# nikhil-lalgudi/distributed-llm-alignment

Measured on AMD Instinct MI355X. Metric: preference-samples/sec (whole node), Llama-3-8B DPO at 1/2/4/8 MI355X, higher is better.
Workload: dtype bf16; 1 GPU; model=llama3-8b, global_batch=16, seq_len=1024, parallelism=dp1, micro_batch_pairs=4, grad_accum=4, ref_model=frozen, co-resident, backend=single-process, gemm_selection=tunableop:off

## Files before the change

### distributed_llm_alignment_amd/csrc/attention.hip

```cpp
#include <cstdlib>
#include <stdexcept>
#include <type_traits>
#include "common.h"

#include <cstring>
#include "attn_params.h"

namespace dla {

typedef __attribute__((address_space(3))) s16x4 lds_s16x4;

template <int D>
constexpr int attn_dp() { return (D + 31) / 32 * 32; }

template <int W>
__device__ __forceinline__ int swz(int row, int ch) {
  constexpr int NCH = W / 8;
  constexpr int MASK = (NCH & (NCH - 1)) == 0 ? NCH - 1 : 3;
  const int f = (((row & 3) << 2) | ((row >> 2) & 3)) & MASK;
  return row * W + ((ch ^ f) << 3);
}

__device__ __forceinline__ int ds_swz(int row) { return (row >> 1) & 7; }
__device__ __forceinline__ int ds_off(int row, int c4) { return row * 32 + ((c4 ^ ds_swz(row)) << 2); }
// ... 1232 lines not shown
      bf16_t* dkp = p.dk + b * p.dk_sb + kj * p.dk_st + static_cast<int64_t>(hk) * p.dk_sh;
      bf16_t* dvp = p.dv + b * p.dv_sb + kj * p.dv_st + static_cast<int64_t>(hk) * p.dv_sh;
      auto store_row = [&](bf16_t* dst, f32x16 x, float sc, int dt) {
#pragma unroll
        for (int g4 = 0; g4 < 4; g4 += 2) {
          const uint32_t a0 = pack2bf(x[4 * g4] * sc, x[4 * g4 + 1] * sc);
          const uint32_t a1 = pack2bf(x[4 * g4 + 2] * sc, x[4 * g4 + 3] * sc);
          const uint32_t c0 = pack2bf(x[4 * g4 + 4] * sc, x[4 * g4 + 5] * sc);
          const uint32_t c1 = pack2bf(x[4 * g4 + 6] * sc, x[4 * g4 + 7] * sc);
          const auto r0 = __builtin_amdgcn_permlane32_swap(a0, c0, false, false);
          const auto r1 = __builtin_amdgcn_permlane32_swap(a1, c1, false, false);
          if (32 * dt + 8 * g4 + 8 * h < D)
            *reinterpret_cast<uint4*>(dst + 32 * dt + 8 * g4 + 8 * h) = make_uint4(r0[0], r1[0], r0[1], r1[1]);
        }
      };
      if (D == 80 && p.rope_cos != nullptr) {
        const int pos = p.rope_pos ? p.rope_pos[static_cast<int64_t>(b) * p.Tk + kj] : kj;
        store_row(dkp, unrotate_tile0_rot32(dk[j][0], p.rope_cos + static_cast<int64_t>(pos) * 16 + 4 * h,
                                            p.rope_sin + static_cast<int64_t>(pos) * 16 + 4 * h),
                  p.scale, 0);
#pragma unroll
        for (int dt = 1; dt < DT; ++dt) store_row(dkp, dk[j][dt], p.scale, dt);
      } else if (DP == D && p.rope_cos != nullptr) {
        const int pos = p.rope_pos ? p.rope_pos[static_cast<int64_t>(b) * p.Tk + kj] : kj;
        const float* cp = p.rope_cos + static_cast<int64_t>(pos) * (D / 2) + 4 * h;
        const float* sp = p.rope_sin + static_cast<int64_t>(pos) * (D / 2) + 4 * h;
#pragma unroll
        for (int dt = 0; dt < DT / 2; ++dt) {
          f32x16 lo = dk[j][dt], hi = dk[j][dt + DT / 2];
#pragma unroll
          for (int g = 0; g < 4; ++g) {
            const f32x4 c4 = *reinterpret_cast<const f32x4*>(cp + 32 * dt + 8 * g);
            const f32x4 s4 = *reinterpret_cast<const f32x4*>(sp + 32 * dt + 8 * g);
#pragma unroll
            for (int e = 0; e < 4; ++e) {
              const float a = lo[4 * g + e], bb = hi[4 * g + e];
              lo[4 * g + e] = a * c4[e] + bb * s4[e];
              hi[4 * g + e] = bb * c4[e] - a * s4[e];
            }
          }
          store_row(dkp, lo, p.scale, dt);
          store_row(dkp, hi, p.scale, dt + DT / 2);
        }
      } else {
#pragma unroll
        for (int dt = 0; dt < DT; ++dt) store_row(dkp, dk[j][dt], p.scale, dt);
      }
#pragma unroll
      for (int dt = 0; dt < DT; ++dt) store_row(dvp, dv[j][dt], 1.f, dt);
    } else {
      const int64_t off = ((static_cast<int64_t>(sidx) * p.B + b) * p.Tk + kj) * p.Hkv * D +
                          static_cast<int64_t>(hk) * D;
      float* dkp = p.dk_part + off;
      float* dvp = p.dv_part + off;
#pragma unroll
      for (int dt = 0; dt < DT; ++dt) {
#pragma unroll
        for (int g4 = 0; g4 < 4; ++g4) {
          const int d = 32 * dt + 8 * g4 + 4 * h;
          if (d >= D) continue;
          *reinterpret_cast<f32x4*>(dkp + d) = f32x4{dk[j][dt][4 * g4], dk[j][dt][4 * g4 + 1],
                                                     dk[j][dt][4 * g4 + 2], dk[j][dt][4 * g4 + 3]};
          *reinterpret_cast<f32x4*>(dvp + d) = f32x4{dv[j][dt][4 * g4], dv[j][dt][4 * g4 + 1],
                                                     dv[j][dt][4 * g4 + 2], dv[j][dt][4 * g4 + 3]};
        }
      }
    }
  }
}

#ifdef DLA_BWD_TRACE
__device__ long long g_bwd_trace[8 * 64 * 8];
#define BWD_TS(k)                                                                         \
  do {                                                                                    \
    if (blockIdx.x == DLA_BWD_TRACE && lane == 0 && it < 64)                              \
      g_bwd_trace[(w * 64 + it) * 8 + (k)] = static_cast<long long>(__builtin_amdgcn_s_memtime()); \
  } while (0)
#else
#define BWD_TS(k) \
  do {            \
  } while (0)
#endif

template <int D, bool CAUSAL>
__global__ __launch_bounds__(512) void attn_bwd8_kernel(AttnBwdParams p) {
  constexpr int BKV = kAttnBwdKeys, BQ = kAttnBwdQRows, NT = 512;
  constexpr int DP = attn_dp<D>();
  constexpr int NCH = DP / 8;
  constexpr int NCHL = D / 8;
  constexpr int KS = D / 16;
  constexpr int DT = DP / 32;
  constexpr int NDS = D / 16;
  constexpr bool Q_EXACT = BQ * NCH == NT;
  static_assert(BQ * NCH <= NT && (BKV * NCH) % NT == 0 && BKV == 256 && BQ == 32, "tile geometry");
  __shared__ __attribute__((aligned(16))) bf16_t lds[2 * BQ * DP + BKV * BQ + 2 * BKV * DP];
  bf16_t* const Qs = lds;
  bf16_t* const dOs = lds + BQ * DP;
  bf16_t* const dSs = lds + 2 * BQ * DP;
  bf16_t* const Ks = dSs + BKV * BQ;
  bf16_t* const Vs = Ks + BKV * DP;

  const int tid = threadIdx.x, lane = tid & 63, w = __builtin_amdgcn_readfirstlane(tid >> 6);
  const int l32 = lane & 31, h = lane >> 5;
  const int group = p.Hq / p.Hkv;
  const int hpb = group / p.hsplit;
  const int nrest = p.Hkv * p.B * p.hsplit;
  const int kb = static_cast<int>(blockIdx.x) / nrest;
  int rest = static_cast<int>(blockIdx.x) - kb * nrest;
  const int sidx = rest % p.hsplit;
  rest /= p.hsplit;
  const int hk = rest % p.Hkv, b = rest / p.Hkv;
  const int k0 = kb * BKV;
  const int kw = k0 + 32 * w;
  const int kbeg = p.kv_start ? p.kv_start[b] : 0;
  const int kend = p.kv_end ? p.kv_end[b] : p.Tk;

  const bool rope_in = p.rope_inputs != 0;
  {
    const bf16_t* kp = p.k + b * p.k_sb + static_cast<int64_t>(hk) * p.k_sh;
    const bf16_t* vp = p.v + b * p.v_sb + static_cast<int64_t>(hk) * p.v_sh;
#pragma unroll 2
    for (int c = 0; c < BKV * NCH / NT; ++c) {
      const int ci = tid + NT * c;
      const int row = ci / NCH, ch = ci % NCH;
      const int key = k0 + row;
      const bool in = key < p.Tk && ch < NCHL;
      bf16x8 kv = in ? load_bf16x8(kp + key * p.k_st + ch * 8) : bf16x8{};
      if constexpr (DP == D) {
        if (rope_in)
          kv = rope_rot_chunk<NCH>(kv, ch, in, static_cast<int64_t>(b) * p.Tk + key, key, p.rope_cos,
                                   p.rope_sin, p.rope_pos);
      }
      store_bf16x8(Ks + swz<DP>(row, ch), kv);
      store_bf16x8(Vs + swz<DP>(row, ch), in ? load_bf16x8(vp + key * p.v_st + ch * 8) : bf16x8{});
    }
  }

  int qt0, qend;
  bwd_q_range<CAUSAL>(k0, p.Tq, p.causal_off, p.window, qt0, qend);
  const int nqt = (qend - qt0 + BQ - 1) / BQ;
  const bool block_has_keys = k0 < kend && k0 + BKV > kbeg;
  const int n_iter = block_has_keys ? hpb * nqt : 0;
  const int hq0 = hk * group + sidx * hpb;

  const int qrow = tid / NCH, qch = tid % NCH;
  const bool qslot = (Q_EXACT || tid < BQ * NCH) && qch < NCHL;
  const uint32_t qlo = static_cast<uint32_t>(qrow * p.q_st + qch * 8) * 2u;
  const uint32_t dlo = static_cast<uint32_t>(qrow * p.do_st + qch * 8) * 2u;
  bf16x8 qreg, dreg;
  auto gld = [](const bf16_t* base, uint32_t off) {
    return load_bf16x8(reinterpret_cast<const bf16_t*>(reinterpret_cast<const char*>(base) + off));
  };
  const int qtend = qt0 + nqt * BQ;
  auto advance = [&](int& hq, int& qt) {
    qt += BQ;
    if (qt >= qtend) {
      qt = qt0;
      ++hq;
    }
  };
  auto prefetch = [&](int hq, int qt) {
    const bf16_t* qp = p.q + b * p.q_sb + static_cast<int64_t>(hq) * p.q_sh;
    const bf16_t* dop = p.dout + b * p.do_sb + static_cast<int64_t>(hq) * p.do_sh;
    if (!qslot) {
      qreg = bf16x8{};
      dreg = bf16x8{};
    } else if (qt + BQ <= p.Tq) {
      qreg = gld(qp + static_cast<int64_t>(qt) * p.q_st, qlo);
      dreg = gld(dop + static_cast<int64_t>(qt) * p.do_st, dlo);
    } else {
      const int qq = min(qt + qrow, p.Tq - 1);
      const bf16x8 a = load_bf16x8(qp + qq * p.q_st + qch * 8);
      const bf16x8 g = load_bf16x8(dop + qq * p.do_st + qch * 8);
      const bool in = qt + qrow < p.Tq;
      qreg = in ? a : bf16x8{};
      dreg = in ? g : bf16x8{};
    }
  };
  auto stage = [&]() {
    if (Q_EXACT || tid < BQ * NCH) {
      store_bf16x8(Qs + swz<DP>(qrow, qch), qreg);
      store_bf16x8(dOs + swz<DP>(qrow, qch), dreg);
    }
  };

  const int i16 = lane & 15, qq = i16 >> 2, pp = i16 & 3, half16 = (lane >> 4) & 1, g4l = lane >> 4;
  constexpr int FMASK = (NCH & (NCH - 1)) == 0 ? NCH - 1 : 3;
  auto swzf = [](int row) { return (((row & 3) << 2) | ((row >> 2) & 3)) & FMASK; };
  int rq = l32 * DP, rx = h ^ swzf(l32);
  const int c1 = 2 * half16 + (pp >> 1);
  int tq0 = (4 * h + qq) * DP + (pp & 1) * 4, tx0 = c1 ^ swzf(4 * h + qq);
  int tq1 = (4 * h + 8 + qq) * DP + (pp & 1) * 4, tx1 = c1 ^ swzf(4 * h + 8 + qq);
  int wq = l32 * 32, wx = h ^ ds_swz(l32);
  constexpr int DQT = NDS == 4 ? 1 : 2;
  const int dslice = NDS == 4 ? (w & 3) : w;
  const int dthalf = NDS == 4 ? (w >> 2) : 0;
  int qoff[DQT][2], koff[2];
#pragma unroll
  for (int t = 0; t < DQT; ++t) {
    const int tt = NDS == 4 ? dthalf : t;
    qoff[t][0] = ds_off(8 * g4l + qq, 4 * tt + pp);
    qoff[t][1] = ds_off(8 * g4l + 4 + qq, 4 * tt + pp);
  }
  {
    const int ch = 2 * dslice + (pp >> 1), sub = (pp & 1) * 4;
    koff[0] = swz<DP>(8 * g4l + qq, ch) + sub;
    koff[1] = swz<DP>(8 * g4l + 4 + qq, ch) + sub;
  }

  const int* se = p.seg_end ? p.seg_end + static_cast<int64_t>(b) * p.Tk : nullptr;
  int kse = 0x7fffffff, kse_lo = 0x7fffffff, kse_hi = 0x7fffffff;
  if (se) {
    kse = se[min(kw + l32, p.Tk - 1)];
    kse_lo = __builtin_amdgcn_readfirstlane(se[min(kw, p.Tk - 1)]);
    kse_hi = __builtin_amdgcn_readfirstlane(se[min(kw + 31, p.Tk - 1)]);
  }

  f32x16 dk[DT], dv[DT];
#pragma unroll
  for (int dt = 0; dt < DT; ++dt) {
    dk[dt] = f32x16{};
    dv[dt] = f32x16{};
  }

  float rlse = 0.f, rdel = 0.f;
  auto load_rows = [&](int hq, int qt) {
    const int64_t rb = (static_cast<int64_t>(b) * p.Hq + hq) * p.Tq;
    const int r = min(qt + l32, p.Tq - 1);
    rlse = p.lse2[rb + r];
    rdel = p.delta[rb + r];
  };
  const s16x8 ones = __builtin_bit_cast(s16x8, u32x4{h ? 0u : 0x3F803F80u, 0u, 0u, 0u});
  const float inv_s2 = 1.f / p.scale2;

  int hq = hq0, qt = qt0;
  int hq_r = hq0, qt_r = qt0;
  int hq_p = hq0, qt_p = qt0;
  if (n_iter > 0) {
    prefetch(hq_p, qt_p);
    stage();
    load_rows(hq_r, qt_r);
    advance(hq_p, qt_p);
    if (n_iter > 1) prefetch(hq_p, qt_p);
    advance(hq_p, qt_p);
  }
  __syncthreads();

  if (w >= 4) __builtin_amdgcn_s_setprio(1);
  for (int it = 0; it < n_iter; ++it) {
    advance(hq_r, qt_r);
    asm volatile("" : "+v"(rq), "+v"(rx), "+v"(tq0), "+v"(tx0), "+v"(tq1), "+v"(tx1), "+v"(wq), "+v"(wx));
    auto roff = [&](int s) { return rq + (((2 * s) ^ rx) << 3); };
    auto toff = [&](int dt, int r) { return r ? tq1 + (((4 * dt) ^ tx1) << 3) : tq0 + (((4 * dt) ^ tx0) << 3); };
    BWD_TS(0);

    bool act = kw < kend && kw + 32 > kbeg && qt < kse_hi;
    bool need_mask = kw < kbeg || kw + 32 > kend || qt + BQ > p.Tq || qt + BQ > kse_lo;
    if (CAUSAL) {
      act = act && kw <= qt + BQ - 1 + p.causal_off;
      need_mask = need_mask || (kw + 31 > qt + p.causal_off);
      if (p.window > 0) {
        act = act && (kw + 31 > qt + p.causal_off - p.window);
        need_mask = need_mask || (kw <= qt + BQ - 1 + p.causal_off - p.window);
      }
    }

    s16x8 sb0 = s16x8{}, sb1 = s16x8{};
    if (act) {
      f32x16 sacc = f32x16{}, dpacc = f32x16{};
      const bf16_t* Kw = Ks + 32 * w * DP;
      const bf16_t* Vw = Vs + 32 * w * DP;
      s16x8 fa[2], fb[2];
      auto chain = [&](const bf16_t* A, const bf16_t* Bm, f32x16& acc) {
        fa[0] = *reinterpret_cast<const s16x8*>(A + roff(0));
        fb[0] = *reinterpret_cast<const s16x8*>(Bm + roff(0));
#pragma unroll
        for (int s = 0; s < KS; ++s) {
          if (s + 1 < KS) {
            fa[(s + 1) & 1] = *reinterpret_cast<const s16x8*>(A + roff(s + 1));
            fb[(s + 1) & 1] = *reinterpret_cast<const s16x8*>(Bm + roff(s + 1));
          }
          __builtin_amdgcn_sched_barrier(0);
          acc = mfma32(fa[s & 1], fb[s & 1], acc);
          __builtin_amdgcn_sched_barrier(0);
        }
      };
      chain(Qs, Kw, sacc);
      chain(dOs, Vw, dpacc);
      {
        const bool rv = qt + l32 < p.Tq;
        float x = -rlse * inv_s2;
        x = (rv && __builtin_isfinite(x)) ? x : -1e30f;
        const float y = rv ? -rdel : 0.f;
        const float xh = bf2f(static_cast<bf16_t>(pack2bf(x, 0.f) & 0xffffu));
        const float yh = bf2f(static_cast<bf16_t>(pack2bf(y, 0.f) & 0xffffu));
        const s16x8 ax = __builtin_bit_cast(s16x8, u32x4{h ? 0u : pack2bf(x, x - xh), 0u, 0u, 0u});
        const s16x8 ay = __builtin_bit_cast(s16x8, u32x4{h ? 0u : pack2bf(y, y - yh), 0u, 0u, 0u});
        sacc = mfma32(ax, ones, sacc);
        dpacc = mfma32(ay, ones, dpacc);
      }
      BWD_TS(1);
      const int kj = kw + l32;
      int lo = 0, hi = min(p.Tq, kse) - qt - 4 * h;
      if (kj < kbeg || kj >= kend) hi = 0;
      if (CAUSAL) {
        const int dlt = kj - qt - p.causal_off - 4 * h;
        lo = max(lo, dlt);
        if (p.window > 0) hi = min(hi, dlt + p.window);
      }
      const unsigned span = hi > lo ? static_cast<unsigned>(hi - lo) : 0u;
#pragma unroll
      for (int i = 0; i < 16; ++i) sacc[i] = ex2(sacc[i] * p.scale2);
      if (need_mask) {
#pragma unroll
        for (int i = 0; i < 16; ++i) {
          const int rr = (i & 3) + 8 * (i >> 2);
          sacc[i] = static_cast<unsigned>(rr - lo) < span ? sacc[i] : 0.f;
        }
      }
#pragma unroll
      for (int i = 0; i < 16; ++i) dpacc[i] = sacc[i] * dpacc[i];
      const s16x8 pb0 = pack8(sacc, 0), pb1 = pack8(sacc, 8);
      sb0 = pack8(dpacc, 0);
      sb1 = pack8(dpacc, 8);
      BWD_TS(2);
      s16x8 ta[2], tb[2], tc[2], td[2];
      auto ld_kv = [&](int dt, int sl) {
        const int o0 = toff(dt, 0), o1 = toff(dt, 1);
        ta[sl] = cat4(tr_read(dOs + o0), tr_read(dOs + o1));
        tb[sl] = cat4(tr_read(dOs + 16 * DP + o0), tr_read(dOs + 16 * DP + o1));
        tc[sl] = cat4(tr_read(Qs + o0), tr_read(Qs + o1));
        td[sl] = cat4(tr_read(Qs + 16 * DP + o0), tr_read(Qs + 16 * DP + o1));
      };
      ld_kv(0, 0);
      __builtin_amdgcn_sched_barrier(0);
#pragma unroll
      for (int dt = 0; dt < DT; ++dt) {
        if (dt + 1 < DT) ld_kv(dt + 1, (dt + 1) & 1);
        __builtin_amdgcn_sched_barrier(0);
        dv[dt] = mfma32(ta[dt & 1], pb0, dv[dt]);
        dk[dt] = mfma32(tc[dt & 1], sb0, dk[dt]);
        dv[dt] = mfma32(tb[dt & 1], pb1, dv[dt]);
        dk[dt] = mfma32(td[dt & 1], sb1, dk[dt]);
        __builtin_amdgcn_sched_barrier(0);
      }
      BWD_TS(3);
    }
    {
      const u32x4 ds0 = __builtin_bit_cast(u32x4, sb0), ds1 = __builtin_bit_cast(u32x4, sb1);
      bf16_t* dSw = dSs + 32 * w * 32;
      *reinterpret_cast<uint2*>(dSw + wq + ((0 ^ wx) << 2)) = make_uint2(ds0[0], ds0[1]);
      *reinterpret_cast<uint2*>(dSw + wq + ((2 ^ wx) << 2)) = make_uint2(ds0[2], ds0[3]);
      *reinterpret_cast<uint2*>(dSw + wq + ((4 ^ wx) << 2)) = make_uint2(ds1[0], ds1[1]);
      *reinterpret_cast<uint2*>(dSw + wq + ((6 ^ wx) << 2)) = make_uint2(ds1[2], ds1[3]);
    }
    BWD_TS(4);
    __syncthreads();
    BWD_TS(5);

    if (it + 1 < n_iter) {
      stage();
      if (it + 2 < n_iter) prefetch(hq_p, qt_p);
      load_rows(hq_r, qt_r);
    }
    BWD_TS(6);
    if (w < NDS || NDS == 4) {
      f32x4 acc[DQT];
#pragma unroll
      for (int t = 0; t < DQT; ++t) acc[t] = f32x4{0.f, 0.f, 0.f, 0.f};
      constexpr int NB = 3, NKS = BKV / 32;
      s16x8 kf[NB], af[NB][DQT];
      auto ld_dq = [&](int ks, int sl) {
        kf[sl] = cat4(tr_read(Ks + 32 * ks * DP + koff[0]), tr_read(Ks + 32 * ks * DP + koff[1]));
#pragma unroll
        for (int t = 0; t < DQT; ++t)
          af[sl][t] = cat4(tr_read(dSs + 32 * ks * 32 + qoff[t][0]), tr_read(dSs + 32 * ks * 32 + qoff[t][1]));
      };
      ld_dq(0, 0);
      ld_dq(1, 1);
#pragma unroll
      for (int ks = 0; ks < NKS; ++ks) {
        if (ks + 2 < NKS) ld_dq(ks + 2, (ks + 2) % NB);
        __builtin_amdgcn_sched_barrier(0);
#pragma unroll
        for (int t = 0; t < DQT; ++t)
          acc[t] = __builtin_amdgcn_mfma_f32_16x16x32_bf16(af[ks % NB][t], kf[ks % NB], acc[t], 0, 0, 0);
        __builtin_amdgcn_sched_barrier(0);
      }
      const int64_t rs = static_cast<int64_t>(p.Hq) * D;
      const int64_t sbase = ((static_cast<int64_t>(kb) * p.B + b) * p.slab_rows + qt) * rs +
                            static_cast<int64_t>(hq) * D + 16 * dslice;
      const uint32_t so = static_cast<uint32_t>(4 * g4l * rs + i16);
      if (p.dq_slab16 != nullptr) {
        bf16_t* sp = p.dq_slab16 + sbase;
#pragma unroll
        for (int t = 0; t < DQT; ++t) {
          const int tt = NDS == 4 ? dthalf : t;
#pragma unroll
          for (int e = 0; e < 4; ++e) sp[(16 * tt + e) * rs + so] = f2bf(acc[t][e] * p.scale);
        }
      } else {
        char* sp = reinterpret_cast<char*>(p.dq_slab + sbase);
#pragma unroll
        for (int t = 0; t < DQT; ++t) {
          const int tt = NDS == 4 ? dthalf : t;
#pragma unroll
          for (int e = 0; e < 4; ++e)
            *reinterpret_cast<float*>(sp + ((16 * tt + e) * rs + so) * 4u) = acc[t][e] * p.scale;
        }
      }
    }
    BWD_TS(7);
    __syncthreads();
    advance(hq, qt);
    advance(hq_p, qt_p);
  }

  const int kj = kw + l32;
  if (kj >= p.Tk) return;
  if (p.hsplit == 1) {
    bf16_t* dkp = p.dk + b * p.dk_sb + kj * p.dk_st + static_cast<int64_t>(hk) * p.dk_sh;
    bf16_t* dvp = p.dv + b * p.dv_sb + kj * p.dv_st + static_cast<int64_t>(hk) * p.dv_sh;
    auto store_row = [&](bf16_t* dst, f32x16 x, float sc, int dt) {
#pragma unroll
      for (int g4 = 0; g4 < 4; g4 += 2) {
        const uint32_t a0 = pack2bf(x[4 * g4] * sc, x[4 * g4 + 1] * sc);
        const uint32_t a1 = pack2bf(x[4 * g4 + 2] * sc, x[4 * g4 + 3] * sc);
        const uint32_t c0 = pack2bf(x[4 * g4 + 4] * sc, x[4 * g4 + 5] * sc);
        const uint32_t c1 = pack2bf(x[4 * g4 + 6] * sc, x[4 * g4 + 7] * sc);
// ... 302 lines not shown
  return prev;
}

template <int D, int HP>
static void fwd_launch(const AttnParams& p0, bool causal, hipStream_t st) {
  constexpr int NW = 8, BQ = 32 * NW / HP;
  AttnParams p = p0;
  {
    const AttnFwdSwitches& sw = attn_fwd_switches();
    p.fwd_prio = sw.prio;
    p.fwd_sgpr = sw.sgpr;
    p.fwd_pro = sw.pro;
    p.fwd_ostage = sw.ostage;
    p.fwd_msub = sw.msub;
  }
  const int nqb = (p.Tq + BQ - 1) / BQ;
  const int64_t nblk = static_cast<int64_t>(nqb) * (p.Hq / HP) * p.B;
  if (fwd_persist(p.Tk) && nblk < (int64_t(1) << 30)) {
    const int grid = static_cast<int>(std::min<int64_t>(nblk, device_cus()));
    if (causal) attn_fwd_persist_kernel<D, true, NW, HP><<<grid, 64 * NW, 0, st>>>(p, static_cast<int>(nblk));
    else attn_fwd_persist_kernel<D, false, NW, HP><<<grid, 64 * NW, 0, st>>>(p, static_cast<int>(nblk));
    return;
  }
  const dim3 grid(static_cast<unsigned>(nblk));
  if constexpr (D == 128) {
    if (p.fwd_msub) {
      if (causal) attn_fwd_kernel<D, true, NW, HP, true><<<grid, 64 * NW, 0, st>>>(p);
      else attn_fwd_kernel<D, false, NW, HP, true><<<grid, 64 * NW, 0, st>>>(p);
      return;
    }
  }
  if (causal) attn_fwd_kernel<D, true, NW, HP><<<grid, 64 * NW, 0, st>>>(p);
  else attn_fwd_kernel<D, false, NW, HP><<<grid, 64 * NW, 0, st>>>(p);
}

template <int D>
static void fwd_dispatch(const AttnParams& p, bool causal, hipStream_t st) {
  static const int forced = [] {
    const char* e = std::getenv("DLA_ATTN_FWD_HP");
    return e ? std::atoi(e) : 0;
  }();
  const int group = p.Hq / p.Hkv;
  const int want = forced > 0 ? forced : 4;
  if (want >= 4 && group % 4 == 0) fwd_launch<D, 4>(p, causal, st);
  else if (want >= 2 && group % 2 == 0) fwd_launch<D, 2>(p, causal, st);
  else fwd_launch<D, 1>(p, causal, st);
}

void launch_attn_fwd(const AttnParams& p, int D, bool causal, hipStream_t st) {
  if (p.B == 0 || p.Tq == 0) return;
  switch (D) {
    case 64: fwd_dispatch<64>(p, causal, st); break;
    case 80: fwd_dispatch<80>(p, causal, st); break;
    case 128: fwd_dispatch<128>(p, causal, st); break;
    default: throw std::invalid_argument("attn_fwd: head_dim must be 64, 80 or 128");
  }
}

void launch_attn_bwd_delta(const bf16_t* o, const bf16_t* dout, int64_t o_sb, int64_t o_st,
                           int64_t o_sh, int64_t do_sb, int64_t do_st, int64_t do_sh, int B,
                           int H, int T, int D, float* delta, hipStream_t st) {
  const int64_t rows = static_cast<int64_t>(B) * H * T;
  if (rows == 0) return;
  const int64_t rows_per_block = 4 * (64 / (D <= 64 ? 8 : 16));
  const unsigned nb = static_cast<unsigned>((rows + rows_per_block - 1) / rows_per_block);
  attn_bwd_delta_kernel<<<nb, 256, 0, st>>>(o, dout, o_sb, o_st, o_sh, do_sb, do_st, do_sh, B, H, T, D, delta);
}

static int attn_bwd_waves() {
  const char* e = std::getenv("DLA_ATTN_BWD_WAVES");
  return (e && std::atoi(e) == 4) ? 4 : 8;
}

bool attn_dq_slab_bf16() {
  const char* e = std::getenv("DLA_ATTN_DQ_BF16");
  return attn_bwd_waves() == 8 && !(e && std::atoi(e) == 0);
}

bool attn_dkv_part_bf16() {
  const char* e = std::getenv("DLA_ATTN_DKV_BF16");
  return attn_bwd_waves() == 8 && !(e && std::atoi(e) == 0);
}

template <int D>
static void bwd_dispatch(const AttnBwdParams& p_in, bool causal, hipStream_t st) {
  const AttnBwdParams& p = p_in;
  const int nkb = (p.Tk + kAttnBwdKeys - 1) / kAttnBwdKeys;
  const dim3 grid(nkb * p.Hkv * p.B * p.hsplit);
  if (attn_bwd_waves() == 8) {
    if (causal) attn_bwd8_kernel<D, true><<<grid, 512, 0, st>>>(p);
    else attn_bwd8_kernel<D, false><<<grid, 512, 0, st>>>(p);
    return;
  }
  if (causal) attn_bwd_kernel<D, true><<<grid, 256, 0, st>>>(p);
  else attn_bwd_kernel<D, false><<<grid, 256, 0, st>>>(p);
}

void launch_attn_bwd(const AttnBwdParams& p, int D, bool causal, hipStream_t st) {
  if (p.B == 0 || p.Tq == 0 || p.Tk == 0) return;
  switch (D) {
    case 64: bwd_dispatch<64>(p, causal, st); break;
    case 80: bwd_dispatch<80>(p, causal, st); break;
    case 128: bwd_dispatch<128>(p, causal, st); break;
    default: throw std::invalid_argument("attn_bwd: head_dim must be 64, 80 or 128");
  }
}

void launch_attn_dq_reduce(const float* slab, int nkb, int B, int Tq, int slab_rows, int Hq, int D,
                           bool causal, int causal_off, int window, const int* kv_start,
                           const int* kv_end, int Tk, bf16_t* dst, int64_t d_sb, int64_t d_st,
                           int64_t d_sh, const float* rcos, const float* rsin, const int* rpos,
                           int rot, hipStream_t st, const bf16_t* slab16) {
  const int64_t work = static_cast<int64_t>(B) * Tq * Hq * (rcos ? rot / 16 + (D - rot) / 8 : D / 8);
  if (work == 0) return;
  if (slab16 != nullptr) {
    if (causal)
      attn_dq_reduce_kernel<true, bf16_t><<<stream_grid(work), 256, 0, st>>>(
          slab16, nkb, B, Tq, slab_rows, Hq, D, causal_off, window, kv_start, kv_end, Tk, dst, d_sb, d_st, d_sh,
          rcos, rsin, rpos, rot);
    else
      attn_dq_reduce_kernel<false, bf16_t><<<stream_grid(work), 256, 0, st>>>(
          slab16, nkb, B, Tq, slab_rows, Hq, D, causal_off, window, kv_start, kv_end, Tk, dst, d_sb, d_st, d_sh,
          rcos, rsin, rpos, rot);
    return;
  }
  if (causal)
    attn_dq_reduce_kernel<true><<<stream_grid(work), 256, 0, st>>>(
        slab, nkb, B, Tq, slab_rows, Hq, D, causal_off, window, kv_start, kv_end, Tk, dst, d_sb, d_st, d_sh,
        rcos, rsin, rpos, rot);
  else
    attn_dq_reduce_kernel<false><<<stream_grid(work), 256, 0, st>>>(
        slab, nkb, B, Tq, slab_rows, Hq, D, causal_off, window, kv_start, kv_end, Tk, dst, d_sb, d_st, d_sh,
        rcos, rsin, rpos, rot);
}

void launch_attn_dkv_reduce(const float* dkp, const float* dvp, int hs, int B, int Tk, int Hkv,
                            int D, float scale, bf16_t* dk, int64_t dk_sb, int64_t dk_st,
                            int64_t dk_sh, bf16_t* dv, int64_t dv_sb, int64_t dv_st,
                            int64_t dv_sh, const float* rcos, const float* rsin, const int* rpos,
                            int rot, hipStream_t st, const bf16_t* dkp16, const bf16_t* dvp16) {
  const int64_t work = static_cast<int64_t>(B) * Tk * Hkv * (rcos ? rot / 16 + (D - rot) / 8 : D / 8);
  if (work == 0) return;
  if (dkp16 != nullptr) {
    attn_dkv_reduce_kernel<bf16_t><<<stream_grid(work), 256, 0, st>>>(
        dkp16, dvp16, hs, B, Tk, Hkv, D, scale, dk, dk_sb, dk_st, dk_sh, dv, dv_sb, dv_st, dv_sh, rcos, rsin,
        rpos, rot);
    return;
  }
  attn_dkv_reduce_kernel<float><<<stream_grid(work), 256, 0, st>>>(dkp, dvp, hs, B, Tk, Hkv, D, scale, dk,
                                                                   dk_sb, dk_st, dk_sh, dv, dv_sb, dv_st,
                                                                   dv_sh, rcos, rsin, rpos, rot);
}

}
```

### distributed_llm_alignment_amd/csrc/attn_params.h

```cpp
#pragma once
#include <stdint.h>

namespace dla {

using bf16_t = uint16_t;

struct AttnParams {
  const bf16_t* q;
  const bf16_t* k;
  const bf16_t* v;
  bf16_t* o;
  float* lse2;
  int64_t q_sb, q_st, q_sh;
  int64_t k_sb, k_st, k_sh;
  int64_t v_sb, v_st, v_sh;
  int64_t o_sb, o_st, o_sh;
  int B, Hq, Hkv, Tq, Tk;
  float scale2;
  int causal_off;
  int window;
  const int* kv_start;
  const int* kv_end;
  const int* seg_start;
  const float* rope_cos;
  const float* rope_sin;
  const int* rope_pos;
  int rope_k;
  bf16_t* q_rot;
  int64_t qr_sb, qr_st, qr_sh;
  int fwd_prio;
  int fwd_sgpr;
  int fwd_pro;
  int fwd_ostage;
  int fwd_msub;
  unsigned long long* stamps;
};

constexpr int kAttnBwdKeys = 256;
constexpr int kAttnBwdQRows = 32;

struct AttnBwdParams {
  const bf16_t* q;
  const bf16_t* k;
  const bf16_t* v;
  const bf16_t* dout;
  const float* lse2;
  const float* delta;
  float* dq_slab;
  bf16_t* dq_slab16;
  float* dk_part;
  float* dv_part;
  bf16_t* dk_part16;
  bf16_t* dv_part16;
  bf16_t* dk;
  bf16_t* dv;
  int hsplit;
  int slab_rows;
  int64_t q_sb, q_st, q_sh;
  int64_t k_sb, k_st, k_sh;
  int64_t v_sb, v_st, v_sh;
  int64_t do_sb, do_st, do_sh;
  int64_t dk_sb, dk_st, dk_sh;
  int64_t dv_sb, dv_st, dv_sh;
  int B, Hq, Hkv, Tq, Tk;
  float scale;
  float scale2;
  int causal_off;
  int window;
  const int* kv_start;
  const int* kv_end;
  const int* seg_end;
  const float* rope_cos;
  const float* rope_sin;
  const int* rope_pos;
  int rope_inputs;
  int rope_rot;
};

}
```

### distributed_llm_alignment_amd/csrc/bindings.cpp

```cpp
#include <ATen/ATen.h>
#include <ATen/hip/impl/HIPGuardImplMasqueradingAsCUDA.h>
#include <ATen/hip/impl/HIPStreamMasqueradingAsCUDA.h>
#include <torch/library.h>

#include <hip/hip_runtime_api.h>

#include <algorithm>
#include <cstdint>
#include <cstdlib>
#include <tuple>

#include "attn_params.h"
#include "bind_util.h"

namespace dla {

void launch_norm_fwd(const bf16_t*, const bf16_t*, bf16_t*, const bf16_t*, const bf16_t*, bf16_t*,
                     float*, float*, int, int, float, bool, hipStream_t);
void launch_norm_bwd(const bf16_t*, const bf16_t*, const bf16_t*, const float*, const float*,
                     const bf16_t*, bf16_t*, float*, float*, bf16_t*, bf16_t*, int, int, bool,
                     hipStream_t);
int norm_bwd_grid(int rows);
int norm_wgrad_scratch_rows();
void launch_swiglu_fwd(const bf16_t*, bf16_t*, int64_t, int, hipStream_t);
void launch_swiglu_bwd(const bf16_t*, const bf16_t*, bf16_t*, int64_t, int, hipStream_t);
void launch_swiglu_fwd_t(const bf16_t*, bf16_t*, bf16_t*, int64_t, int, hipStream_t);
void launch_swiglu_bwd_t(const bf16_t*, const bf16_t*, bf16_t*, bf16_t*, int64_t, int, hipStream_t);
void launch_gelu_fwd(const bf16_t*, bf16_t*, int64_t, hipStream_t);
void launch_gelu_bwd(const bf16_t*, const bf16_t*, bf16_t*, int64_t, hipStream_t);
void launch_rope_fwd(const bf16_t*, int64_t, bf16_t*, bf16_t*, const float*, const float*,
                     const int*, int64_t, int, int, int, int, int, int, hipStream_t);
void launch_rope_bwd(const bf16_t*, const bf16_t*, bf16_t*, int64_t, const float*, const float*,
                     const int*, int64_t, int, int, int, int, int, int, hipStream_t);
void launch_logprob_fwd(const bf16_t*, int64_t, int, int64_t, int64_t, const int64_t*, float*,
                        float*, hipStream_t);
void launch_logprob_bwd(bf16_t*, int64_t, int, int64_t, int64_t, const int64_t*, const float*,
                        const float*, hipStream_t);
void launch_row_lse(const bf16_t*, int64_t, int, int64_t, float*, hipStream_t);
bool launch_logprob_bwd_t(bf16_t*, int64_t, int, int64_t, int64_t, const int64_t*, const float*,
                          const float*, bf16_t*, hipStream_t);
void launch_logprob_entropy_fwd(const bf16_t*, int64_t, int, int64_t, int64_t, const int64_t*, float*,
                                float*, float*, hipStream_t);
void launch_logprob_entropy_bwd(bf16_t*, int64_t, int, int64_t, int64_t, const int64_t*, const float*,
                                const float*, const float*, const float*, hipStream_t);
bool launch_logprob_entropy_bwd_t(bf16_t*, int64_t, int, int64_t, int64_t, const int64_t*, const float*,
                                  const float*, const float*, const float*, bf16_t*, hipStream_t);
void launch_ensemble_kl(bf16_t*, const bf16_t*, int64_t, int64_t, int, int, const float*,
                        const float*, int64_t, const float*, float*, bool, hipStream_t);
void launch_seq_reduce(const float*, const float*, int, int, float*, float*, hipStream_t);
void launch_seq_expand_grad(const float*, const float*, const float*, int, int, bool, float*,
                            hipStream_t);
void launch_dpo_loss(const float*, const float*, int, float, float, float*, float*, float*,
                     float*, hipStream_t);
void launch_pairwise_loss(const float*, const float*, int, float*, float*, float*, float*,
                          hipStream_t);
void launch_kl_penalty_pg(const float*, const float*, const float*, int, float, float*, float*,
                          float*, float*, hipStream_t);
void launch_gae(const float*, const float*, const float*, int, int, float, float, float*, float*,
                hipStream_t);
void launch_ppo_policy_loss(const float*, const float*, const float*, const float*, int64_t, float,
                            float*, float*, float*, hipStream_t);
void launch_ppo_value_loss(const float*, const float*, const float*, const float*, int64_t, float,
                           float*, float*, hipStream_t);
void launch_group_advantages(const float*, int, int, bool, float, float*, float*, hipStream_t);
void launch_grpo_loss(const float*, const float*, const float*, const float*, const float*,
                      const float*, int, int, float, float, float, int, float, float*, float*,
                      float*, float*, hipStream_t);
void launch_adamw(bf16_t*, float*, const void*, bool, float*, float*, int64_t, float, float,
                  float, float, float, int, const float*, float, hipStream_t);
void launch_grad_sumsq(const void*, bool, int64_t, float*, float*, bool, hipStream_t);
int sumsq_grid(int64_t n);
void launch_clip_coef(const float*, float, float*, float*, hipStream_t);

void launch_attn_fwd(const AttnParams&, int, bool, hipStream_t);
int attn_fwd_set_switch(const char* name, int value);
void launch_attn_bwd_delta(const bf16_t*, const bf16_t*, int64_t, int64_t, int64_t, int64_t,
                           int64_t, int64_t, int, int, int, int, float*, hipStream_t);
void launch_attn_bwd(const AttnBwdParams&, int, bool, hipStream_t);
bool attn_dkv_part_bf16();
bool attn_dq_slab_bf16();
void launch_attn_dq_reduce(const float*, int, int, int, int, int, int, bool, int, int,
                           const int*, const int*, int, bf16_t*, int64_t, int64_t, int64_t,
                           const float*, const float*, const int*, int, hipStream_t, const bf16_t*);
void launch_attn_dkv_reduce(const float*, const float*, int, int, int, int, int, float, bf16_t*,
                            int64_t, int64_t, int64_t, bf16_t*, int64_t, int64_t, int64_t,
                            const float*, const float*, const int*, int, hipStream_t, const bf16_t*,
                            const bf16_t*);
void launch_transpose_bf16(const bf16_t*, int64_t, int64_t, int64_t, bf16_t*, int64_t, hipStream_t);

std::tuple<at::Tensor, at::Tensor, at::Tensor, at::Tensor> norm_fwd(
    const at::Tensor& x, const c10::optional<at::Tensor>& res, const at::Tensor& w,
    const c10::optional<at::Tensor>& b, double eps, bool rms) {
  check_bf16(x, "x");
  check_bf16(w, "w");
  TORCH_CHECK(x.is_contiguous(), "x must be contiguous");
  const int64_t H = x.size(-1);
  TORCH_CHECK(H % 8 == 0 && H <= 8192, "norm_fwd: hidden size must be a multiple of 8 and <= 8192");
  TORCH_CHECK(w.numel() == H && w.is_contiguous(), "w shape");
  const int64_t rows = x.numel() / H;
  TORCH_CHECK(rows < (1ll << 31), "too many rows");
  c10::hip::HIPGuardMasqueradingAsCUDA g(x.device());
  auto y = at::empty_like(x);
  at::Tensor so;
  const bf16_t* rptr = nullptr;
  if (res && res->defined()) {
    check_bf16(*res, "res");
    TORCH_CHECK(res->sizes() == x.sizes() && res->is_contiguous(), "res shape");
    so = at::empty_like(x);
    rptr = cbp(*res);
  }
  const bf16_t* bptr = nullptr;
  if (b && b->defined()) {
    check_bf16(*b, "b");
    TORCH_CHECK(b->numel() == H && b->is_contiguous(), "b shape");
    bptr = cbp(*b);
  }
  auto opt = x.options().dtype(at::kFloat);
  auto rstd = at::empty({rows}, opt);
  auto mean = rms ? at::empty({0}, opt) : at::empty({rows}, opt);
  check_aligned16(x, "x");
  launch_norm_fwd(cbp(x), rptr, so.defined() ? bp(so) : nullptr, cbp(w), bptr, bp(y),
                  rstd.data_ptr<float>(), rms ? nullptr : mean.data_ptr<float>(),
                  static_cast<int>(rows), static_cast<int>(H), static_cast<float>(eps), rms,
                  cur_stream(x));
  return {y, so.defined() ? so : at::empty({0}, x.options()), rstd, mean};
}

std::tuple<at::Tensor, at::Tensor, at::Tensor> norm_bwd(const at::Tensor& dy, const at::Tensor& s,
                                                        const at::Tensor& w,
                                                        const at::Tensor& rstd,
                                                        const c10::optional<at::Tensor>& mean,
                                                        const c10::optional<at::Tensor>& dres,
                                                        bool has_bias, bool rms) {
  check_bf16(dy, "dy");
  check_bf16(s, "s");
  check_bf16(w, "w");
  check_f32(rstd, "rstd");
  TORCH_CHECK(dy.is_contiguous() && s.is_contiguous() && dy.sizes() == s.sizes(), "dy/s shape");
  const int64_t H = s.size(-1);
  const int64_t rows = s.numel() / H;
  TORCH_CHECK(H % 8 == 0 && H <= 16384, "hidden size");
  TORCH_CHECK(rstd.numel() == rows, "rstd shape");
  const float* mptr = nullptr;
  if (!rms) {
    TORCH_CHECK(mean && mean->defined() && mean->numel() == rows, "LayerNorm needs mean");
    mptr = mean->data_ptr<float>();
  }
  const bf16_t* dr = nullptr;
  if (dres && dres->defined()) {
    check_bf16(*dres, "dres");
    TORCH_CHECK(dres->sizes() == s.sizes() && dres->is_contiguous(), "dres shape");
    dr = cbp(*dres);
  }
  c10::hip::HIPGuardMasqueradingAsCUDA g(s.device());
  auto ds = at::empty_like(s);
  const int grid = norm_bwd_grid(static_cast<int>(rows));
  auto fopt = s.options().dtype(at::kFloat);
  const int srows = grid + norm_wgrad_scratch_rows();
  auto dwp = at::empty({srows, H}, fopt);
  auto dbp = has_bias ? at::empty({srows, H}, fopt) : at::empty({0}, fopt);
  auto dw = at::empty({H}, w.options());
  auto db = has_bias ? at::empty({H}, w.options()) : at::empty({0}, w.options());
  launch_norm_bwd(cbp(dy), cbp(s), cbp(w), rstd.data_ptr<float>(), mptr, dr, bp(ds),
// ... 247 lines not shown
  p.o_sb = o.stride(0); p.o_st = o.stride(1); p.o_sh = o.stride(2);
  p.B = B; p.Hq = Hq; p.Hkv = Hkv; p.Tq = Tq; p.Tk = Tk;
  p.scale2 = static_cast<float>(scale * 1.4426950408889634);
  p.causal_off = static_cast<int>(causal_off);
  p.window = static_cast<int>(window);
  p.kv_start = (kv_start && kv_start->defined()) ? kv_start->data_ptr<int>() : nullptr;
  p.kv_end = (kv_end && kv_end->defined()) ? kv_end->data_ptr<int>() : nullptr;
  p.seg_start = seg_ptr(segs, B, Tq, Tk, causal, causal_off, q, 0);
  rope_args(rope_cos, rope_sin, rope_pos, q, B, Tq, Tk, D, causal_off, &p.rope_cos, &p.rope_sin,
            &p.rope_pos);
  TORCH_CHECK(p.rope_cos == nullptr || D != 80, "RoPE on load: full-rotary head dims 64 / 128 only");
  p.rope_k = rope_k ? 1 : 0;
  if (q_rot && q_rot->defined()) {
    TORCH_CHECK(p.rope_cos != nullptr, "q_rot needs the rotary tables");
    check_bthd(*q_rot, "q_rot");
    TORCH_CHECK(q_rot->sizes() == q.sizes(), "q_rot shape");
    same_device(q, *q_rot);
    p.q_rot = bp(*q_rot);
    p.qr_sb = q_rot->stride(0); p.qr_st = q_rot->stride(1); p.qr_sh = q_rot->stride(2);
  }
  static const bool stamps = [] {
    const char* e = std::getenv("DLA_ATTN_STAMPS");
    return e != nullptr && std::atoi(e) == 1;
  }();
  if (stamps) {
    auto& buf = attn_stamp_buffer();
    if (!buf.defined() || buf.device() != q.device())
      buf = at::zeros({1024 * 8 * 4}, q.options().dtype(at::kLong));
    p.stamps = reinterpret_cast<unsigned long long*>(buf.data_ptr<int64_t>());
  }
  launch_attn_fwd(p, static_cast<int>(D), causal, cur_stream(q));
  return {o, lse2};
}

static int device_cus(int dev) {
  static int cache[64] = {0};
  if (dev < 0 || dev >= 64) return 256;
  if (cache[dev] == 0) {
    int n = 0;
    if (hipDeviceGetAttribute(&n, hipDeviceAttributeMultiprocessorCount, dev) != hipSuccess || n <= 0) n = 256;
    cache[dev] = n;
  }
  return cache[dev];
}

static int attn_bwd_hsplit(int64_t nkb, int64_t Hkv, int64_t B, int64_t group, bool causal, int cus) {
  const int64_t base = nkb * Hkv * B;
  const int64_t target = causal ? 2 * static_cast<int64_t>(cus) : cus;
  int hs = 1;
  while (base * hs < target && group % (2 * hs) == 0) hs *= 2;
  return hs;
}

void attn_bwd(const at::Tensor& dout, const at::Tensor& q, const at::Tensor& k,
              const at::Tensor& v, const at::Tensor& o, const at::Tensor& lse2, at::Tensor& dq,
              at::Tensor& dk, at::Tensor& dv, double scale, bool causal, int64_t causal_off,
              int64_t window, const c10::optional<at::Tensor>& kv_start,
              const c10::optional<at::Tensor>& kv_end, const c10::optional<at::Tensor>& segs,
              const c10::optional<at::Tensor>& rope_cos, const c10::optional<at::Tensor>& rope_sin,
              const c10::optional<at::Tensor>& rope_pos, bool rope_inputs) {
  check_bthd(dout, "dout");
  check_bthd(q, "q");
  check_bthd(k, "k");
  check_bthd(v, "v");
  check_bthd(o, "o");
  check_bthd(dq, "dq");
  check_bthd(dk, "dk");
  check_bthd(dv, "dv");
  check_f32(lse2, "lse2");
  const int64_t B = q.size(0), Tq = q.size(1), Hq = q.size(2), D = q.size(3);
  const int64_t Tk = k.size(1), Hkv = k.size(2);
  TORCH_CHECK(D == 64 || D == 80 || D == 128, "head_dim must be 64, 80 or 128");
  TORCH_CHECK(dout.sizes() == q.sizes() && o.sizes() == q.sizes() && dq.sizes() == q.sizes(),
              "dout/o/dq shape");
  TORCH_CHECK(dk.sizes() == k.sizes() && dv.sizes() == v.sizes(), "dk/dv shape");
  TORCH_CHECK(lse2.is_contiguous() && lse2.numel() == B * Hq * Tq, "lse2 shape");
  TORCH_CHECK(Hkv > 0 && Hq % Hkv == 0, "GQA ratio");
  check_kv_range(kv_start, B, "kv_start");
  check_kv_range(kv_end, B, "kv_end");
  c10::hip::HIPGuardMasqueradingAsCUDA g(q.device());
  auto st = cur_stream(q);
  auto fopt = q.options().dtype(at::kFloat);
  auto delta = at::empty({B, Hq, Tq}, fopt);
  launch_attn_bwd_delta(cbp(o), cbp(dout), o.stride(0), o.stride(1), o.stride(2),
                        dout.stride(0), dout.stride(1), dout.stride(2), B, Hq, Tq, D,
                        delta.data_ptr<float>(), st);
  const int64_t nkb = (Tk + kAttnBwdKeys - 1) / kAttnBwdKeys;
  const int64_t slab_rows = (Tq + kAttnBwdQRows - 1) / kAttnBwdQRows * kAttnBwdQRows;
  const bool slab16 = attn_dq_slab_bf16();
  auto slab = at::empty({std::max<int64_t>(nkb, 1), B, slab_rows, Hq, D}, slab16 ? q.options() : fopt);
  const int hs = attn_bwd_hsplit(nkb, Hkv, B, Hq / Hkv, causal, device_cus(q.get_device()));
  at::Tensor dkp, dvp;
  const bool part16 = hs > 1 && attn_dkv_part_bf16();
  if (hs > 1) {
    dkp = at::empty({hs, B, Tk, Hkv, D}, part16 ? q.options() : fopt);
    dvp = at::empty({hs, B, Tk, Hkv, D}, part16 ? q.options() : fopt);
  }
  AttnBwdParams p{};
  p.q = cbp(q); p.k = cbp(k); p.v = cbp(v); p.dout = cbp(dout);
  p.lse2 = lse2.data_ptr<float>(); p.delta = delta.data_ptr<float>();
  p.dq_slab = slab16 ? nullptr : slab.data_ptr<float>();
  p.dq_slab16 = slab16 ? bp(slab) : nullptr;
  p.dk_part = hs > 1 && !part16 ? dkp.data_ptr<float>() : nullptr;
  p.dv_part = hs > 1 && !part16 ? dvp.data_ptr<float>() : nullptr;
  p.dk_part16 = part16 ? bp(dkp) : nullptr;
  p.dv_part16 = part16 ? bp(dvp) : nullptr;
  p.dk = bp(dk); p.dv = bp(dv);
  p.hsplit = hs;
  p.slab_rows = static_cast<int>(slab_rows);
  p.q_sb = q.stride(0); p.q_st = q.stride(1); p.q_sh = q.stride(2);
  p.k_sb = k.stride(0); p.k_st = k.stride(1); p.k_sh = k.stride(2);
  p.v_sb = v.stride(0); p.v_st = v.stride(1); p.v_sh = v.stride(2);
  p.do_sb = dout.stride(0); p.do_st = dout.stride(1); p.do_sh = dout.stride(2);
  p.dk_sb = dk.stride(0); p.dk_st = dk.stride(1); p.dk_sh = dk.stride(2);
  p.dv_sb = dv.stride(0); p.dv_st = dv.stride(1); p.dv_sh = dv.stride(2);
  p.B = B; p.Hq = Hq; p.Hkv = Hkv; p.Tq = Tq; p.Tk = Tk;
  p.scale = static_cast<float>(scale);
  p.scale2 = static_cast<float>(scale * 1.4426950408889634);
  p.causal_off = static_cast<int>(causal_off);
  p.window = static_cast<int>(window);
  p.kv_start = (kv_start && kv_start->defined()) ? kv_start->data_ptr<int>() : nullptr;
  p.kv_end = (kv_end && kv_end->defined()) ? kv_end->data_ptr<int>() : nullptr;
  p.seg_end = seg_ptr(segs, B, Tq, Tk, causal, causal_off, q, 1);
  rope_args(rope_cos, rope_sin, rope_pos, q, B, Tq, Tk, D, causal_off, &p.rope_cos, &p.rope_sin,
            &p.rope_pos, &p.rope_rot);
  TORCH_CHECK(!rope_inputs || p.rope_cos != nullptr, "rope_inputs needs the rotary tables");
  TORCH_CHECK(!rope_inputs || p.rope_rot == D, "rope_inputs (RoPE on load): full rotary only");
  p.rope_inputs = rope_inputs ? 1 : 0;
  launch_attn_bwd(p, static_cast<int>(D), causal, st);
  launch_attn_dq_reduce(p.dq_slab, static_cast<int>(nkb), static_cast<int>(B), static_cast<int>(Tq),
                        p.slab_rows, static_cast<int>(Hq), static_cast<int>(D), causal, p.causal_off, p.window,
                        p.kv_start, p.kv_end, static_cast<int>(Tk), bp(dq), dq.stride(0),
                        dq.stride(1), dq.stride(2), p.rope_cos, p.rope_sin, p.rope_pos, p.rope_rot, st,
                        p.dq_slab16);
  if (hs > 1) {
    launch_attn_dkv_reduce(p.dk_part, p.dv_part, hs, static_cast<int>(B), static_cast<int>(Tk),
                           static_cast<int>(Hkv), static_cast<int>(D), p.scale, bp(dk),
                           dk.stride(0), dk.stride(1), dk.stride(2), bp(dv), dv.stride(0),
                           dv.stride(1), dv.stride(2), p.rope_cos, p.rope_sin, p.rope_pos, p.rope_rot, st,
                           p.dk_part16, p.dv_part16);
  }
}

void transpose_bf16(const at::Tensor& in, at::Tensor& out) {
  check_bf16(in, "in");
  check_bf16(out, "out");
  TORCH_CHECK(in.dim() == 2 && out.dim() == 2 && in.stride(1) == 1 && out.stride(1) == 1 &&
                  out.size(0) == in.size(1) && out.size(1) == in.size(0),
              "transpose_bf16: in [R, C], out [C, R], unit column stride");
  TORCH_CHECK(in.stride(0) % 8 == 0 && out.stride(0) % 8 == 0, "16-byte aligned rows");
  check_aligned16(in, "in");
  check_aligned16(out, "out");
  same_device(in, out);
  c10::hip::HIPGuardMasqueradingAsCUDA g(in.device());
  launch_transpose_bf16(cbp(in), in.size(0), in.size(1), in.stride(0), bp(out), out.stride(0),
                        cur_stream(in));
}

static void check_logits(const at::Tensor& logits) {
  check_bf16(logits, "logits");
  TORCH_CHECK(logits.dim() == 2 && logits.stride(1) == 1, "logits must be [N, V] row-major");
}

std::tuple<at::Tensor, at::Tensor> logprob_fwd(const at::Tensor& logits, const at::Tensor& tgt,
                                               int64_t vocab_offset) {
  check_logits(logits);
  TORCH_CHECK(tgt.scalar_type() == at::kLong && tgt.is_contiguous() && tgt.numel() == logits.size(0),
              "targets int64 [N]");
  same_device(logits, tgt);
  c10::hip::HIPGuardMasqueradingAsCUDA g(logits.device());
  auto opt = logits.options().dtype(at::kFloat);
  auto logp = at::empty({logits.size(0)}, opt);
  auto lse = at::empty({logits.size(0)}, opt);
  launch_logprob_fwd(cbp(logits), logits.stride(0), static_cast<int>(logits.size(1)),
                     vocab_offset, logits.size(0), tgt.data_ptr<int64_t>(), logp.data_ptr<float>(),
                     lse.data_ptr<float>(), cur_stream(logits));
  return {logp, lse};
}

void logprob_bwd(at::Tensor& logits, const at::Tensor& tgt, const at::Tensor& lse,
                 const at::Tensor& grad, int64_t vocab_offset) {
  check_logits(logits);
  check_f32(lse, "lse");
// ... 489 lines not shown
```

Before: 10.14 preference_pairs/s.

## Compute attention-backward delta inside the 8-wave bwd kernel for head_dim 128

Removes the separate delta pre-pass kernel for head_dim 128. The backward kernel now also loads O alongside dO during its Q/dO prefetch, computes rowsum(O·dO) with a DPP cross-lane reduction, writes it to the delta buffer, and reads it back for the next tile's rows. This saves a kernel launch and a separate full pass over O and dO. In exchange, every key-block recomputes delta redundantly, adds one more global load per prefetch, and relies on workgroup-scope ordering between the publish and the later read.

Result: no change. 10.20 preference_pairs/s (median of 6 runs) (+0.6%).

```diff
diff --git a/distributed_llm_alignment_amd/csrc/attention.hip b/distributed_llm_alignment_amd/csrc/attention.hip
--- a/distributed_llm_alignment_amd/csrc/attention.hip
+++ b/distributed_llm_alignment_amd/csrc/attention.hip
@@ -1338,7 +1338,19 @@
   } while (0)
 #endif
 
-template <int D, bool CAUSAL>
+template <int CTRL>
+__device__ __forceinline__ float dpp_f32(float v) {
+  return __int_as_float(__builtin_amdgcn_update_dpp(0, __float_as_int(v), CTRL, 0xf, 0xf, false));
+}
+__device__ __forceinline__ float row16_sum(float x) {
+  x += dpp_f32<0xB1>(x);
+  x += dpp_f32<0x4E>(x);
+  x += dpp_f32<0x141>(x);
+  x += dpp_f32<0x140>(x);
+  return x;
+}
+
+template <int D, bool CAUSAL, bool FDELTA = false>
 __global__ __launch_bounds__(512) void attn_bwd8_kernel(AttnBwdParams p) {
   constexpr int BKV = kAttnBwdKeys, BQ = kAttnBwdQRows, NT = 512;
   constexpr int DP = attn_dp<D>();
@@ -1349,6 +1361,7 @@
   constexpr int NDS = D / 16;
   constexpr bool Q_EXACT = BQ * NCH == NT;
   static_assert(BQ * NCH <= NT && (BKV * NCH) % NT == 0 && BKV == 256 && BQ == 32, "tile geometry");
+  static_assert(!FDELTA || (Q_EXACT && NCH == 16 && DP == D), "in-kernel delta: one DPP row per query row");
   __shared__ __attribute__((aligned(16))) bf16_t lds[2 * BQ * DP + BKV * BQ + 2 * BKV * DP];
   bf16_t* const Qs = lds;
   bf16_t* const dOs = lds + BQ * DP;
@@ -1404,6 +1417,7 @@
   const uint32_t qlo = static_cast<uint32_t>(qrow * p.q_st + qch * 8) * 2u;
   const uint32_t dlo = static_cast<uint32_t>(qrow * p.do_st + qch * 8) * 2u;
   bf16x8 qreg, dreg;
+  [[maybe_unused]] bf16x8 oreg;
   auto gld = [](const bf16_t* base, uint32_t off) {
     return load_bf16x8(reinterpret_cast<const bf16_t*>(reinterpret_cast<const char*>(base) + off));
   };
@@ -1418,12 +1432,16 @@
   auto prefetch = [&](int hq, int qt) {
     const bf16_t* qp = p.q + b * p.q_sb + static_cast<int64_t>(hq) * p.q_sh;
     const bf16_t* dop = p.dout + b * p.do_sb + static_cast<int64_t>(hq) * p.do_sh;
+    [[maybe_unused]] const bf16_t* op = nullptr;
+    if constexpr (FDELTA) op = p.o + b * p.do_sb + static_cast<int64_t>(hq) * p.do_sh;
     if (!qslot) {
       qreg = bf16x8{};
       dreg = bf16x8{};
+      if constexpr (FDELTA) oreg = bf16x8{};
     } else if (qt + BQ <= p.Tq) {
       qreg = gld(qp + static_cast<int64_t>(qt) * p.q_st, qlo);
       dreg = gld(dop + static_cast<int64_t>(qt) * p.do_st, dlo);
+      if constexpr (FDELTA) oreg = gld(op + static_cast<int64_t>(qt) * p.do_st, dlo);
     } else {
       const int qq = min(qt + qrow, p.Tq - 1);
       const bf16x8 a = load_bf16x8(qp + qq * p.q_st + qch * 8);
@@ -1431,6 +1449,7 @@
       const bool in = qt + qrow < p.Tq;
       qreg = in ? a : bf16x8{};
       dreg = in ? g : bf16x8{};
+      if constexpr (FDELTA) oreg = load_bf16x8(op + qq * p.do_st + qch * 8);
     }
   };
   auto stage = [&]() {
@@ -1438,6 +1457,15 @@
       store_bf16x8(Qs + swz<DP>(qrow, qch), qreg);
       store_bf16x8(dOs + swz<DP>(qrow, qch), dreg);
     }
+  };
+  [[maybe_unused]] auto publish = [&](int hq_s, int qt_s) {
+    float acc = 0.f;
+#pragma unroll
+    for (int j = 0; j < 8; ++j) acc += bf2f(oreg[j]) * bf2f(dreg[j]);
+    acc = row16_sum(acc);
+    if (qch == 0 && qt_s + qrow < p.Tq)
+      __hip_atomic_store(p.delta_w + (static_cast<int64_t>(b) * p.Hq + hq_s) * p.Tq + qt_s + qrow, acc,
+                         __ATOMIC_RELAXED, __HIP_MEMORY_SCOPE_WORKGROUP);
   };
 
   const int i16 = lane & 15, qq = i16 >> 2, pp = i16 & 3, half16 = (lane >> 4) & 1, g4l = lane >> 4;
@@ -1484,7 +1512,10 @@
     const int64_t rb = (static_cast<int64_t>(b) * p.Hq + hq) * p.Tq;
     const int r = min(qt + l32, p.Tq - 1);
     rlse = p.lse2[rb + r];
-    rdel = p.delta[rb + r];
+    if constexpr (FDELTA)
+      rdel = __hip_atomic_load(p.delta_w + rb + r, __ATOMIC_RELAXED, __HIP_MEMORY_SCOPE_WORKGROUP);
+    else
+      rdel = p.delta[rb + r];
   };
   const s16x8 ones = __builtin_bit_cast(s16x8, u32x4{h ? 0u : 0x3F803F80u, 0u, 0u, 0u});
   const float inv_s2 = 1.f / p.scale2;
@@ -1494,13 +1525,17 @@
   int hq_p = hq0, qt_p = qt0;
   if (n_iter > 0) {
     prefetch(hq_p, qt_p);
+    if constexpr (FDELTA) publish(hq_r, qt_r);
     stage();
-    load_rows(hq_r, qt_r);
+    if constexpr (!FDELTA) load_rows(hq_r, qt_r);
     advance(hq_p, qt_p);
     if (n_iter > 1) prefetch(hq_p, qt_p);
     advance(hq_p, qt_p);
   }
   __syncthreads();
+  if constexpr (FDELTA) {
+    if (n_iter > 0) load_rows(hq_r, qt_r);
+  }
 
   if (w >= 4) __builtin_amdgcn_s_setprio(1);
   for (int it = 0; it < n_iter; ++it) {
@@ -1601,6 +1636,9 @@
         __builtin_amdgcn_sched_barrier(0);
       }
       BWD_TS(3);
+    }
+    if constexpr (FDELTA) {
+      if (it + 1 < n_iter) publish(hq_r, qt_r);
     }
     {
       const u32x4 ds0 = __builtin_bit_cast(u32x4, sb0), ds1 = __builtin_bit_cast(u32x4, sb1);
@@ -2069,11 +2107,26 @@
   return attn_bwd_waves() == 8 && !(e && std::atoi(e) == 0);
 }
 
+bool attn_bwd_fused_delta(int D) {
+  const char* e = std::getenv("DLA_ATTN_BWD_DELTA");
+  return D == 128 && attn_bwd_waves() == 8 && !(e && std::atoi(e) == 0);
+}
+
 template <int D>
 static void bwd_dispatch(const AttnBwdParams& p_in, bool causal, hipStream_t st) {
   const AttnBwdParams& p = p_in;
   const int nkb = (p.Tk + kAttnBwdKeys - 1) / kAttnBwdKeys;
   const dim3 grid(nkb * p.Hkv * p.B * p.hsplit);
+  if (p.delta_w != nullptr) {
+    if constexpr (D == 128) {
+      if (attn_bwd_waves() != 8 || p.o == nullptr)
+        throw std::invalid_argument("attn_bwd: in-kernel delta needs the 8-wave kernel and o");
+      if (causal) attn_bwd8_kernel<D, true, true><<<grid, 512, 0, st>>>(p);
+      else attn_bwd8_kernel<D, false, true><<<grid, 512, 0, st>>>(p);
+      return;
+    }
+    throw std::invalid_argument("attn_bwd: in-kernel delta is built for head_dim 128 only");
+  }
   if (attn_bwd_waves() == 8) {
     if (causal) attn_bwd8_kernel<D, true><<<grid, 512, 0, st>>>(p);
     else attn_bwd8_kernel<D, false><<<grid, 512, 0, st>>>(p);
diff --git a/distributed_llm_alignment_amd/csrc/attn_params.h b/distributed_llm_alignment_amd/csrc/attn_params.h
--- a/distributed_llm_alignment_amd/csrc/attn_params.h
+++ b/distributed_llm_alignment_amd/csrc/attn_params.h
@@ -46,6 +46,8 @@
   const bf16_t* dout;
   const float* lse2;
   const float* delta;
+  float* delta_w;
+  const bf16_t* o;
   float* dq_slab;
   bf16_t* dq_slab16;
   float* dk_part;
diff --git a/distributed_llm_alignment_amd/csrc/bindings.cpp b/distributed_llm_alignment_amd/csrc/bindings.cpp
--- a/distributed_llm_alignment_amd/csrc/bindings.cpp
+++ b/distributed_llm_alignment_amd/csrc/bindings.cpp
@@ -79,6 +79,7 @@
 void launch_attn_bwd(const AttnBwdParams&, int, bool, hipStream_t);
 bool attn_dkv_part_bf16();
 bool attn_dq_slab_bf16();
+bool attn_bwd_fused_delta(int D);
 void launch_attn_dq_reduce(const float*, int, int, int, int, int, int, bool, int, int,
                            const int*, const int*, int, bf16_t*, int64_t, int64_t, int64_t,
                            const float*, const float*, const int*, int, hipStream_t, const bf16_t*);
@@ -492,9 +493,12 @@
   auto st = cur_stream(q);
   auto fopt = q.options().dtype(at::kFloat);
   auto delta = at::empty({B, Hq, Tq}, fopt);
-  launch_attn_bwd_delta(cbp(o), cbp(dout), o.stride(0), o.stride(1), o.stride(2),
-                        dout.stride(0), dout.stride(1), dout.stride(2), B, Hq, Tq, D,
-                        delta.data_ptr<float>(), st);
+  const bool fdelta = attn_bwd_fused_delta(static_cast<int>(D)) && o.stride(0) == dout.stride(0) &&
+                      o.stride(1) == dout.stride(1) && o.stride(2) == dout.stride(2);
+  if (!fdelta)
+    launch_attn_bwd_delta(cbp(o), cbp(dout), o.stride(0), o.stride(1), o.stride(2),
+                          dout.stride(0), dout.stride(1), dout.stride(2), B, Hq, Tq, D,
+                          delta.data_ptr<float>(), st);
   const int64_t nkb = (Tk + kAttnBwdKeys - 1) / kAttnBwdKeys;
   const int64_t slab_rows = (Tq + kAttnBwdQRows - 1) / kAttnBwdQRows * kAttnBwdQRows;
   const bool slab16 = attn_dq_slab_bf16();
@@ -509,6 +513,10 @@
   AttnBwdParams p{};
   p.q = cbp(q); p.k = cbp(k); p.v = cbp(v); p.dout = cbp(dout);
   p.lse2 = lse2.data_ptr<float>(); p.delta = delta.data_ptr<float>();
+  if (fdelta) {
+    p.delta_w = delta.data_ptr<float>();
+    p.o = cbp(o);
+  }
   p.dq_slab = slab16 ? nullptr : slab.data_ptr<float>();
   p.dq_slab16 = slab16 ? bp(slab) : nullptr;
   p.dk_part = hs > 1 && !part16 ? dkp.data_ptr<float>() : nullptr;
```
